# 16lemoing/waldo

Measured on AMD Instinct MI355X. Metric: warped+composited frames/sec at 256x512, 8 layers; fwd+bwd, higher is better.
Workload: dtype f32; 1 GPU; C3: 8 clips x 14 frames per GPU, 8 layers x 4x256x512, 16 TPS control points, fwd+bwd; frames_per_gpu=112, layers=8, height=256, width=512, parallelism=frames sharded x1, no data-path collective

## Files before the change

waldo_amd/csrc/waldo_common.hip.h:

```cpp
#pragma once
#include <hip/hip_runtime.h>
#include <stdint.h>
#include <type_traits>

#include "../../include/waldo_hip.h"
#include "warp_composite_layout.hip.h"

namespace waldo {

void set_error(const char* fmt, ...);
int launch_status(const char* what);
bool debug_option(int option);

void fill_words(void* dst, unsigned word, size_t bytes, hipStream_t st);
void copy_bytes(void* dst, const void* src, size_t bytes, hipStream_t st);

constexpr int kWave = 64;
constexpr int kBlock = 256;

constexpr int kStatusCtx = 0, kStatusPred = 2;

__device__ __forceinline__ int checked_frame(const int64_t* __restrict__ ts, int64_t i, int limit,
                                             int* __restrict__ status, int slot) {
  const int64_t raw = ts[i];
// ... 27 lines not shown
  return kXcds / g;
}
__device__ __forceinline__ bool xcd_decode_banded(unsigned bid, int nA, int nbands, int nT, int inner,
                                                  int& a, int& tile, int& rest) {
  const int tpb = (nT + nbands - 1) / nbands;
  int unit, j;
  if (!xcd_decode(bid, nA * nbands, tpb * inner, unit, j)) return false;
  a = unit / nbands;
  const int t = j / inner;
  rest = j - t * inner;
  tile = (unit - a * nbands) * tpb + t;
  return tile < nT;
}
__host__ inline int64_t xcd_grid_banded(int64_t nA, int nbands, int64_t nT, int64_t inner) {
  return xcd_grid(nA * nbands, ((nT + nbands - 1) / nbands) * inner);
}

struct Taps {
  float w00, w01, w10, w11;
  uint32_t o00, o01, o10, o11;
  float fx, fy;
  float vx0, vx1, vy0, vy1;
  int x0, y0;
};

__device__ __forceinline__ float unnormalize(float c, int size) {
  return ((c + 1.0f) * (float)size - 1.0f) * 0.5f;
}

struct TapCore {
// ... 330 lines not shown
```

waldo_amd/csrc/warp_composite_bwd_px16.hip.h:

```cpp
#pragma once

namespace waldo {

__device__ __forceinline__ int pk_max_u16(int a, int b) {
  typedef unsigned short u2 __attribute__((ext_vector_type(2)));
  u2 x, y;
  __builtin_memcpy(&x, &a, 4);
  __builtin_memcpy(&y, &b, 4);
  u2 r = __builtin_elementwise_max(x, y);
  int o;
  __builtin_memcpy(&o, &r, 4);
  return o;
}

__device__ __forceinline__ int exponent_of(float v) { return (int)(__float_as_uint(v) >> 23) & 0xff; }

#ifndef WALDO_K1_STAGE_AHEAD
#define WALDO_K1_STAGE_AHEAD 3
#endif

template <int LP>
struct Px16Cfg {
  static constexpr int K3 = kGmapK3, KS = (K3 + 3) / 4;
  static constexpr int NC = 2 * LP, NT = (NC + 15) / 16, GGC = NT * 16, TP = GGC + 1;
// ... 15 lines not shown
  static constexpr int kStage1 = kBtEnd > kStage0 ? kBtEnd : kStage0;
  static constexpr int kStage2 = (!kPark && kAccFloats > kStage1) ? kAccFloats : kStage1;
  static constexpr int kStageFloats = (kStage2 + 3) / 4 * 4;
  static constexpr int kLdsFloats = kParkFloats + kStageFloats + 4 * GGC * 2 + 4 * LP;
  static constexpr int kWavesPerSimd = LP <= 8 ? 3 : 2;
};

template <int LP, bool EXL, bool GOCC, typename TL = float, bool DET = false>
__global__ __launch_bounds__(kBlock, (GOCC ? 2 : Px16Cfg<LP>::kWavesPerSimd)) void warp_composite_bwd_px16_kernel(
    const TL* __restrict__ layers, const float* __restrict__ basis_t,
    const float* __restrict__ mapping, const float* __restrict__ occ,
    const float* __restrict__ grad_rgb, const float* __restrict__ grad_alpha,
    float4* __restrict__ rec, int* __restrict__ cellbox,
    unsigned* __restrict__ cellbound, float* __restrict__ gmap_partial, float* __restrict__ grad_occ,
    int F, int Lrt, int H, int W, int frames_per_block, int ntx, int ntiles, int nchunks, int nbands,
    int ncx, int ncells, float delta) {
  typedef float f32x4 __attribute__((ext_vector_type(4)));
  using C = Px16Cfg<LP>;
  constexpr int K3 = C::K3, KS = C::KS, NT = C::NT, GGC = C::GGC, TP = C::TP, OP = C::OP;
  constexpr bool kPark = C::kPark;
  const int L = EXL ? LP : Lrt;
  const int64_t HW = (int64_t)H * W;
  const int lane = threadIdx.x & (kWave - 1), wave = __builtin_amdgcn_readfirstlane(threadIdx.x >> 6);
  const int arow = lane & 15, kk = lane >> 4;
  int chunk, tile, rest_;
  if (!xcd_decode_banded(blockIdx.x, nchunks, nbands, ntiles, 1, chunk, tile, rest_)) return;

  __shared__ __attribute__((aligned(16))) float lds[C::kLdsFloats];
  float* park = lds;
  float* img = lds + C::kParkFloats;
  float* gg = kPark ? park : img;
  float* boxred = img + C::kStageFloats;
  int* wbound = reinterpret_cast<int*>(boxred + 4 * GGC * 2);
  const int pix = threadIdx.x;

  const int col0 = (tile % ntx) * kLdsTile, row0 = (tile / ntx) * kLdsTile + wave * 4;
  const bool live = col0 + arow < W && row0 + kk < H;
  const float livef = live ? 1.0f : 0.0f;
  const int64_t p = (int64_t)min(row0 + kk, H - 1) * W + min(col0 + arow, W - 1);
  for (int i = threadIdx.x; i < C::kStageFloats; i += kBlock) img[i] = 0.0f;

  float av[4][KS];
#pragma unroll
  for (int g = 0; g < 4; ++g) {
    const uint32_t pa = (uint32_t)(min(row0 + g, H - 1) * W + min(col0 + arow, W - 1));
#pragma unroll
    for (int ks = 0; ks < KS; ++ks) {
      const int k = 4 * ks + kk;
      const float bs = ldb(basis_t, ((uint32_t)min(k, K3 - 1) * (uint32_t)HW + pa) * 4u);
      av[g][ks] = (k < K3) ? bs : 0.0f;
    }
  }
  __syncthreads();

  const float half_size = 0.5f * (float)((arow & 1) ? H : W);
  const float half_size_m1 = 0.5f * (float)(((arow & 1) ? H : W) - 1);
  const int f0 = chunk * frames_per_block;
  const int f1 = min(F, f0 + frames_per_block);
  const int lane_k = lane, arow_k = arow, kk_k = kk, pix_k = pix;
  for (int f = f0; f < f1; ++f) {
    int lane = lane_k, arow = arow_k, kk = kk_k, pix = pix_k;
    asm volatile("" : "+v"(lane), "+v"(arow), "+v"(kk), "+v"(pix));
    const float* oc = occ + (int64_t)f * L * L;
    f32x4 acc[4][NT];
#pragma unroll
    for (int g = 0; g < 4; ++g)
#pragma unroll
      for (int nt = 0; nt < NT; ++nt) acc[g][nt] = (f32x4){0.0f, 0.0f, 0.0f, 0.0f};
    const float* mp = mapping + (int64_t)f * L * K3 * 2;
    {
      float mraw[KS][NT];
#pragma unroll
      for (int ks = 0; ks < KS; ++ks)
// ... 98 lines not shown
        bw[l] = ((xmax - bx0[l] + 1) + 3) & ~3;
        bh[l] = ymax - ymin + 1;
        fits[l] = bh[l] * bw[l] <= kStageCap;
      }
    }

    WALDO_PRIO_ON(WALDO_K1_PRIO_MASK, 2);
    const float g0 = grad_rgb[(int64_t)f * 3 * HW + p] * livef;
    const float g1 = grad_rgb[(int64_t)f * 3 * HW + HW + p] * livef;
    const float g2 = grad_rgb[(int64_t)f * 3 * HW + 2 * HW + p] * livef;
    const float gsum = fabsf(g0) + fabsf(g1) + fabsf(g2);
    float a[LP], G[LP];
    float dxr[kPark ? 1 : LP], dxa[kPark ? 1 : LP], dyr[kPark ? 1 : LP], dya[kPark ? 1 : LP];

    constexpr int kAhead = LP < WALDO_K1_STAGE_AHEAD ? LP : WALDO_K1_STAGE_AHEAD;
    int item_l = threadIdx.x;
    asm volatile("" : "+v"(item_l));
    typename StageOf<TL>::type stg[LP];
    auto issue = [&](int l) {
      const int lc = EXL ? l : min(l, L - 1);
      const TL* src = layers + ((int64_t)f * L + lc) * 4 * HW;
      const int bw2 = bw[l] >> 1, n = fits[l] ? bh[l] * bw2 : 1;
      const int ox = fits[l] ? __mul24(by0[l], W) + bx0[l] : 0;
      const float rcp = __builtin_amdgcn_rcpf((float)bw2);
      const int item = min(item_l, n - 1);
      const int r = (int)(((float)item + 0.5f) * rcp);
      const int xh = item - __mul24(r, bw2);
      stage_load(stg[l], src, HW, (unsigned)(ox + __mul24(r, W) + 2 * xh));
    };
#pragma unroll
    for (int l = 0; l < kAhead; ++l) issue(l);
    WALDO_PRIO_OFF(WALDO_K1_PRIO_MASK, 2);
    {
#pragma unroll
      for (int l = 0; l < LP; ++l) {
        if (!EXL && l >= L) {
          a[l] = 0.0f;
          G[l] = 0.0f;
          if constexpr (kPark) {
            reinterpret_cast<f32x4*>(park)[l * kBlock + pix] = (f32x4){0.0f, 0.0f, 0.0f, 0.0f};
          } else {
            dxr[l] = dxa[l] = dyr[l] = dya[l] = 0.0f;
          }
          continue;
        }
        WALDO_PRIO_ON(WALDO_K1_PRIO_MASK, 1);
        if (fits[l]) {
          const int n = bh[l] * (bw[l] >> 1);
          if (item_l < n)
            stage_put<TL>(img + (l & 1) * kImgBufFloats, item_l, stg[l]);
        }
        if (l + kAhead < LP) issue(l + kAhead);
        WALDO_PRIO_OFF(WALDO_K1_PRIO_MASK, 1);
        float gal = 0.0f;
        if (grad_alpha != nullptr) gal = grad_alpha[((int64_t)f * L + l) * HW + p];
        __syncthreads();
        const TapCore tc = tap_core_px(gxs[l], gys[l], H, W);
        const float* b0 = img + (l & 1) * kImgBufFloats;
        float sv[4], sx[4], sy[4];
        if (!fits[l]) {
          const Taps tg = finish_taps(tc, H, W);
          const TL* base = layers + ((int64_t)f * L + l) * 4 * HW;
#pragma unroll
          for (int c = 0; c < 4; ++c) sv[c] = tap_sample_d(base + c * HW, tg, sx[c], sy[c], delta);
        } else {
// ... 271 lines not shown
```

waldo_amd/csrc/warp_composite_fwd_lds.hip.h:

```cpp
#pragma once

namespace waldo {

#ifndef WALDO_FWD12_WAVES
#define WALDO_FWD12_WAVES 4
#endif
#ifndef WALDO_FWD8_WAVES
#define WALDO_FWD8_WAVES 3
#endif
#ifndef WALDO_FWD_PRIO_MASK
#define WALDO_FWD_PRIO_MASK 0
#endif
#ifndef WALDO_K1_PRIO_MASK
#define WALDO_K1_PRIO_MASK 3
#endif
#define WALDO_PRIO_ON(mask, bit) do { if ((mask) & (bit)) __builtin_amdgcn_s_setprio(1); } while (0)
#define WALDO_PRIO_OFF(mask, bit) do { if ((mask) & (bit)) __builtin_amdgcn_s_setprio(0); } while (0)
#ifndef WALDO_STAGE_AHEAD
#define WALDO_STAGE_AHEAD 2
#endif

struct BoxTaps {
  float fx, fy;
  float v00, v01, v10, v11;
// ... 15 lines not shown
  p.cs = t.x0 - p.xb;
  p.rs = t.y0 - p.yb;
  return p;
}

__device__ __forceinline__ int block_origin(float i, int size) {
  i = __builtin_amdgcn_fmed3f(i, -2.0f, (float)size + 1.0f);
  return min(max((int)floorf(i), 0), size - 2);
}

typedef float f32x2_t __attribute__((ext_vector_type(2)));
typedef float f32x4_t __attribute__((ext_vector_type(4)));

constexpr int kImgBufFloats = 4 * kStageCap;

struct StageRegs {
  f32x2_t c0, c1, c2, c3;
};

__device__ __forceinline__ f32x2_t pk_lo(f32x2_t a, f32x2_t b) {
  f32x2_t d;
  asm("v_pk_mov_b32 %0, %1, %2 op_sel:[0,0]" : "=v"(d) : "v"(a), "v"(b));
  return d;
}
__device__ __forceinline__ f32x2_t pk_hi(f32x2_t a, f32x2_t b) {
  f32x2_t d;
  asm("v_pk_mov_b32 %0, %1, %2 op_sel:[1,1]" : "=v"(d) : "v"(a), "v"(b));
  return d;
}

__device__ __forceinline__ void stage_store(float* imgbuf, int item, const StageRegs& r) {
  f32x4_t* dst = reinterpret_cast<f32x4_t*>(imgbuf + 8 * item);
  dst[0] = __builtin_shufflevector(pk_lo(r.c0, r.c1), pk_lo(r.c2, r.c3), 0, 1, 2, 3);
  dst[1] = __builtin_shufflevector(pk_hi(r.c0, r.c1), pk_hi(r.c2, r.c3), 0, 1, 2, 3);
}

__device__ __forceinline__ f32x2_t ld8(const float* __restrict__ base, uint32_t byte_off) {
  return *reinterpret_cast<const f32x2_t*>(reinterpret_cast<const char*>(base) + byte_off);
}

struct StageRegs16 {
  uint32_t c0, c1, c2, c3;
};
template <typename T>
struct StageOf {
  typedef StageRegs16 type;
};
template <>
struct StageOf<float> {
  typedef StageRegs type;
};

template <typename T>
__device__ __forceinline__ f32x2_t widen2(uint32_t w) {
  if constexpr (std::is_same_v<T, __bf16>) {
    return (f32x2_t){__uint_as_float(w << 16), __uint_as_float(w & 0xffff0000u)};
  } else {
    typename Half2<T>::type h;
    __builtin_memcpy(&h, &w, 4);
    return __builtin_convertvector(h, f32x2_t);
  }
}

template <typename T>
__device__ __forceinline__ void stage_load(typename StageOf<T>::type& r, const T* __restrict__ src, int64_t HW,
                                           unsigned tex) {
  if constexpr (std::is_same_v<T, float>) {
    const unsigned off = tex * 4u;
    r.c0 = ld8(src, off);
    r.c1 = ld8(src + HW, off);
    r.c2 = ld8(src + 2 * HW, off);
    r.c3 = ld8(src + 3 * HW, off);
  } else {
    auto ld4 = [](const T* base, unsigned byte_off) {
      return *reinterpret_cast<const uint32_t*>(reinterpret_cast<const char*>(base) + byte_off);
    };
    const unsigned off = tex * 2u;
    r.c0 = ld4(src, off);
    r.c1 = ld4(src + HW, off);
    r.c2 = ld4(src + 2 * HW, off);
    r.c3 = ld4(src + 3 * HW, off);
  }
}

template <typename T>
__device__ __forceinline__ void stage_put(float* imgbuf, int item, const typename StageOf<T>::type& r) {
  if constexpr (std::is_same_v<T, float>) {
    stage_store(imgbuf, item, r);
  } else {
    StageRegs w;
    w.c0 = widen2<T>(r.c0);
    w.c1 = widen2<T>(r.c1);
    w.c2 = widen2<T>(r.c2);
    w.c3 = widen2<T>(r.c3);
    stage_store(imgbuf, item, w);
  }
}

struct PairBlock {
  f32x2_t p00[2], p01[2], p10[2], p11[2];
};

__device__ __forceinline__ PairBlock read_block(const float* imgbuf, int idx, int bw) {
  const f32x4_t* r0 = reinterpret_cast<const f32x4_t*>(imgbuf + 4 * idx);
  const f32x4_t* r1 = r0 + bw;
  const f32x4_t t00 = r0[0], t01 = r0[1], t10 = r1[0], t11 = r1[1];
  PairBlock b;
  b.p00[0] = __builtin_shufflevector(t00, t00, 0, 1);
  b.p00[1] = __builtin_shufflevector(t00, t00, 2, 3);
  b.p01[0] = __builtin_shufflevector(t01, t01, 0, 1);
  b.p01[1] = __builtin_shufflevector(t01, t01, 2, 3);
// ... 21 lines not shown

__device__ __forceinline__ f32x2_t lerp2(const f32x2_t p00, const f32x2_t p01, const f32x2_t p10,
                                         const f32x2_t p11, float fx, float fy) {
  const f32x2_t fx2 = {fx, fx}, fy2 = {fy, fy};
  const f32x2_t top = __builtin_elementwise_fma(fx2, p01 - p00, p00);
  const f32x2_t bot = __builtin_elementwise_fma(fx2, p11 - p10, p10);
  return __builtin_elementwise_fma(fy2, bot - top, top);
}

template <int LP, bool EXL, bool FOLD, int NW = 4, typename TL = float>
__global__ __launch_bounds__(NW * kWave, (NW == 8 ? 1 : 1) * (LP <= 8 ? WALDO_FWD8_WAVES : (LP <= 12 ? (EXL ? WALDO_FWD12_WAVES : 3) : 2))) void warp_composite_fwd_lds_kernel(
    const TL* __restrict__ layers, const float* __restrict__ basis_t,
    const float* __restrict__ mapping, const float* __restrict__ inv_kernel,
    const float* __restrict__ src_pts, const float* __restrict__ occ, float* __restrict__ rgb,
    float* __restrict__ alpha_out, int F, int Lrt, int H, int W, int frames_per_block, int ntx,
    int ntiles, int nchunks, int nbands, float delta) {
  typedef float f32x4 __attribute__((ext_vector_type(4)));
  constexpr int K3 = 19, KS = (K3 + 3) / 4;
  constexpr int NC = 2 * LP, NT = (NC + 15) / 16, GGC = NT * 16, TP = GGC + 1;
  constexpr int kThreads = NW * kWave, kCap = kStageCap * NW / 4, kBuf = 4 * kCap;
  constexpr int kImgFloats = 2 * kBuf;
  constexpr int kTFloats = NW * kWave * TP;
  constexpr int kMain = kImgFloats > kTFloats ? kImgFloats : kTFloats;
  const int L = EXL ? LP : Lrt;
  const int64_t HW = (int64_t)H * W;
  const int lane = threadIdx.x & (kWave - 1), wave = __builtin_amdgcn_readfirstlane(threadIdx.x >> 6);
  const int arow = lane & 15, kk = lane >> 4;
  int chunk, tile, rest_;
  if (!xcd_decode_banded(blockIdx.x, nchunks, nbands, ntiles, 1, chunk, tile, rest_)) return;
  const int col0 = (tile % ntx) * (kLdsTile * NW / 4) + (wave >> 2) * kLdsTile;
  const int row0 = (tile / ntx) * kLdsTile + (wave & 3) * 4;
  PixelMap pm;
  pm.live = col0 + arow < W && row0 + kk < H;
  pm.p = (int64_t)min(row0 + kk, H - 1) * W + min(col0 + arow, W - 1);
  const int64_t p = pm.p;

  constexpr int kMapFloats = FOLD ? 2 * LP * K3 * 2 : 0;
  __shared__ __attribute__((aligned(16))) float lds[kMain + NW * GGC * 2 + kMapFloats];
  float* img = lds;
  float* boxred = lds + kMain;
  float* smap = boxred + NW * GGC * 2;
  auto fold_mapping = [&](int fm) {
    if constexpr (FOLD) {
      for (int e = threadIdx.x; e < L * K3 * 2; e += kThreads) {
// ... 38 lines not shown
  };
  static_assert(kMain % 4 == 0, "cleared sixteen bytes at a time");
  for (int i = threadIdx.x; i < kMain / 4; i += kThreads) reinterpret_cast<f32x4*>(lds)[i] = (f32x4){0.0f, 0.0f, 0.0f, 0.0f};

  float av[4][KS];
#pragma unroll
  for (int g = 0; g < 4; ++g) {
    const uint32_t pa = (uint32_t)(min(row0 + g, H - 1) * W + min(col0 + arow, W - 1));
#pragma unroll
    for (int ks = 0; ks < KS; ++ks) {
      const int k = 4 * ks + kk;
      const float bs = ldb(basis_t, ((uint32_t)min(k, K3 - 1) * (uint32_t)HW + pa) * 4u);
      av[g][ks] = (k < K3) ? bs : 0.0f;
    }
  }
  const int f0 = chunk * frames_per_block;
  const int f1 = min(F, f0 + frames_per_block);
  if (f0 < f1) fold_first(f0);
  __syncthreads();

  const float half_size = 0.5f * (float)((arow & 1) ? H : W);
  const float half_size_m1 = 0.5f * (float)(((arow & 1) ? H : W) - 1);
  const int lane_k = lane, arow_k = arow, kk_k = kk;
  for (int f = f0; f < f1; ++f) {
    int lane = lane_k, arow = arow_k, kk = kk_k;
    asm volatile("" : "+v"(lane), "+v"(arow), "+v"(kk));
    f32x4 acc[4][NT];
#pragma unroll
    for (int g = 0; g < 4; ++g)
#pragma unroll
      for (int nt = 0; nt < NT; ++nt) acc[g][nt] = (f32x4){0.0f, 0.0f, 0.0f, 0.0f};
    const float* mp = FOLD ? smap + (f & 1) * (LP * K3 * 2) : mapping + (int64_t)f * L * K3 * 2;
// ... 76 lines not shown
      hi_t[nt] = block_origin(mx, size) + 1;
    }
    int bx0[LP], by0[LP], bw[LP], bh[LP];
#pragma unroll
    for (int l = 0; l < LP; ++l) {
      const int nt = (2 * l) / 16, ln = (2 * l) % 16;
      const int xmin = __builtin_amdgcn_readlane(lo_t[nt], ln), xmax = __builtin_amdgcn_readlane(hi_t[nt], ln);
      const int ymin = __builtin_amdgcn_readlane(lo_t[nt], ln + 1), ymax = __builtin_amdgcn_readlane(hi_t[nt], ln + 1);
      bx0[l] = xmin & ~3;
      by0[l] = ymin;
      bw[l] = ((xmax - bx0[l] + 1) + 3) & ~3;
      bh[l] = ymax - ymin + 1;
    }

    constexpr int kAhead = LP < WALDO_STAGE_AHEAD ? LP : WALDO_STAGE_AHEAD;
    static_assert(kCap / 2 == kThreads, "one box item per lane");
    int item_l = threadIdx.x;
    asm volatile("" : "+v"(item_l));
    float s[LP][4];
    typename StageOf<TL>::type stg[LP];
    auto issue = [&](int l) {
      const int lc = EXL ? l : min(l, L - 1);
      const TL* src = layers + ((int64_t)f * L + lc) * 4 * HW;
      const bool fits = bh[l] * bw[l] <= kCap;
      const int bw2 = bw[l] >> 1, n = fits ? bh[l] * bw2 : 1;
      const int ox = fits ? __mul24(by0[l], W) + bx0[l] : 0;
      const float rcp = __builtin_amdgcn_rcpf((float)bw2);
      const int item = min(item_l, n - 1);
      const int r = (int)(((float)item + 0.5f) * rcp);
      const int xh = item - __mul24(r, bw2);
      stage_load(stg[l], src, HW, (unsigned)(ox + __mul24(r, W) + 2 * xh));
    };
    WALDO_PRIO_ON(WALDO_FWD_PRIO_MASK, 2);
#pragma unroll
    for (int l = 0; l < kAhead; ++l) issue(l);
    WALDO_PRIO_OFF(WALDO_FWD_PRIO_MASK, 2);
    {
#pragma unroll
      for (int l = 0; l < LP; ++l) {
        if (!EXL && l >= L) {
          s[l][0] = s[l][1] = s[l][2] = 0.0f;
          s[l][3] = -1.0f;
          continue;
        }
        const bool fits = bh[l] * bw[l] <= kCap;
        WALDO_PRIO_ON(WALDO_FWD_PRIO_MASK, 1);
        if (fits) {
          const int n = bh[l] * (bw[l] >> 1);
          if (item_l < n)
            stage_put<TL>(img + (l & 1) * kBuf, item_l, stg[l]);
        }
        if (l + kAhead < LP) issue(l + kAhead);
        WALDO_PRIO_OFF(WALDO_FWD_PRIO_MASK, 1);
        __syncthreads();
        if (fits) {
          const TapCore tc = tap_core_px(gx[l], gy[l], H, W);
          const float* b0 = img + (l & 1) * kBuf;
          f32x2_t sv[2];
          if (__ballot(!tap_interior(tc, H, W)) == 0ull) {
            const int idx = __mul24(tc.y0 - by0[l], bw[l]) + (tc.x0 - bx0[l]);
            const PairBlock pb = read_block(b0, idx, bw[l]);
#pragma unroll
            for (int q = 0; q < 2; ++q) sv[q] = lerp2(pb.p00[q], pb.p01[q], pb.p10[q], pb.p11[q], tc.fx, tc.fy);
          } else {
            const BoxTaps t = make_box_taps(tc, H, W);
// ... 67 lines not shown
```

waldo_amd/csrc/warp_composite_kernels.hip.h:

```cpp
#pragma once
#include <stdlib.h>

#include <type_traits>

#include "waldo_common.hip.h"

namespace waldo {

constexpr int kMaxLayers = 32;
constexpr int kMaxK3 = 32;
constexpr int kFwdGroup = 4;
constexpr int kBwdGroup = 2;

template <int K3P, bool EXK>
__device__ __forceinline__ void load_basis(float (&bas)[K3P], const float* __restrict__ basis_t,
                                           int64_t HW, int64_t p, int K3) {
#pragma unroll
  for (int k = 0; k < K3P; ++k) {
    if constexpr (EXK) {
      bas[k] = basis_t[(int64_t)k * HW + p];
    } else {
      const int kc = min(k, K3 - 1);
      const float v = basis_t[(int64_t)kc * HW + p];
      bas[k] = (k < K3) ? v : 0.0f;
// ... 221 lines not shown
        const float ggy = giy * (0.5f * (float)H);
        float part[2 * K3P];
#pragma unroll
        for (int k = 0; k < K3P; ++k) {
          part[2 * k] = bas[k] * ggx;
          part[2 * k + 1] = bas[k] * ggy;
        }
        float red = wave_transpose_reduce<2 * K3P>(part, lane);
        int idx = bitrev6(lane);
        if (idx < 2 * K3) atomicAdd(grad_mapping + ((int64_t)f * L + l) * K3 * 2 + idx, red);
      }
    }
  }
}

constexpr int kRedOut = 32, kRedSlices = kBlock / kRedOut;

static __global__ __launch_bounds__(kBlock) void warp_composite_gmap_reduce_kernel(
    const float* __restrict__ gmap_partial, float* __restrict__ grad_mapping, int F, int L,
    int ntiles, int groups) {
  const int per = L * kGmapK3 * 2;
  const int64_t f = blockIdx.x / groups;
  const int o = (blockIdx.x % groups) * kRedOut + (threadIdx.x % kRedOut);
  const int slice = threadIdx.x / kRedOut;
  __shared__ float red[kRedSlices][kRedOut];
  float s0 = 0.0f, s1 = 0.0f;
  if (o < per) {
    const int t0 = (int)((int64_t)ntiles * slice / kRedSlices), t1 = (int)((int64_t)ntiles * (slice + 1) / kRedSlices);
    const float* src = gmap_partial + f * ntiles * per + o;
    int t = t0;
    for (; t + 1 < t1; t += 2) {
      s0 += src[(int64_t)t * per];
      s1 += src[(int64_t)(t + 1) * per];
    }
    if (t < t1) s0 += src[(int64_t)t * per];
  }
  red[slice][threadIdx.x % kRedOut] = s0 + s1;
  __syncthreads();
  if (slice == 0 && o < per) {
    float sum = 0.0f;
#pragma unroll
    for (int k = 0; k < kRedSlices; ++k) sum += red[k][threadIdx.x];
    grad_mapping[f * per + o] += sum;
  }
}

template <typename T>
void launch_splat(const float* rec, const float* grad_rgb, const int* cellbox,
                  const unsigned* cellbound, T* grad_layers, int F, int L, int H, int W,
                  hipStream_t st);

}

#include "det_common.hip.h"
#include "warp_composite_fwd_lds.hip.h"
#include "warp_composite_bwd_px16.hip.h"

namespace waldo {

static inline int chunk_frames(int F, int64_t ntiles) {
  for (int c = 8; c >= 2; --c) {
    const int chunks = (F + c - 1) / c;
    if (chunks % kXcds == 0 && (int64_t)chunks * ntiles >= 2048) return c;
  }
  return 1;
}

struct TileGeom {
  int ntx, nty, ntiles;
};

static inline TileGeom tile_geom(int H, int W, int rows) {
  TileGeom g;
  g.ntx = (W + kTileW - 1) / kTileW;
  g.nty = (H + rows - 1) / rows;
  g.ntiles = g.ntx * g.nty;
  return g;
}

#ifndef WALDO_FWD_NW
// ... 3 lines not shown
static void launch_fwd(const T* layers, const float* basis_t, const float* mapping,
                       const float* inv_kernel, const float* src_pts,
                       const float* occ, float* rgb, float* alpha, int F, int L, int H, int W,
                       int K3, float delta, hipStream_t st) {
  constexpr bool kF32 = std::is_same_v<T, float>;
  const TileGeom g = tile_geom(H, W, 4);
  const int fpb = chunk_frames(F, g.ntiles);
  const int nchunks = (F + fpb - 1) / fpb;
  const int nbands = xcd_bands(nchunks);
  dim3 grid((unsigned)xcd_grid_banded(nchunks, nbands, g.ntiles, 1));
  if constexpr (EXK) {
    if (!kF32 || (!debug_option(WALDO_DEBUG_FWD_PLAIN) && staged_eligible(H, W))) {
      constexpr int NW = (WALDO_FWD_NW == 8 && LP <= 12) ? 8 : 4;
      constexpr int TW = kLdsTile * NW / 4;
      const int ntx16 = (W + TW - 1) / TW, nt16 = ntx16 * ((H + kLdsTile - 1) / kLdsTile);
      dim3 grid16((unsigned)xcd_grid_banded(nchunks, nbands, nt16, 1));
      auto go = [&](auto exl, auto fold) {
        constexpr bool EXL = decltype(exl)::value, FOLD = decltype(fold)::value;
        hipLaunchKernelGGL((warp_composite_fwd_lds_kernel<LP, EXL, FOLD, NW, T>), grid16, dim3(NW * kWave), 0, st, layers,
                           basis_t, mapping, inv_kernel, src_pts, occ, rgb, alpha, F, L, H, W, fpb, ntx16, nt16,
                           nchunks, nbands, delta);
      };
      using Y = std::true_type;
      using N = std::false_type;
      if (src_pts != nullptr) {
        if (L == LP) go(Y{}, Y{}); else go(N{}, Y{});
      } else {
        if (L == LP) go(Y{}, N{}); else go(N{}, N{});
      }
      return;
    }
  }
  if constexpr (kF32) {
    if (L == LP)
      hipLaunchKernelGGL((warp_composite_fwd_kernel<LP, K3P, true, EXK>), grid, dim3(kBlock), 0, st,
                         layers, basis_t, mapping, occ, rgb, alpha, F, L, H, W, K3, fpb, g.ntx, g.ntiles,
// ... 25 lines not shown
                        int F, int L, int H, int W, float delta, hipStream_t st, float* occ_slab = nullptr) {
  const Bwd2Layout lo = bwd2_layout(F, L, H, W);
  char* ws = reinterpret_cast<char*>(workspace);
  int* boxes = reinterpret_cast<int*>(ws);
  unsigned* bounds = reinterpret_cast<unsigned*>(ws + lo.box_bytes);
  float4* rec = reinterpret_cast<float4*>(ws + lo.box_bytes + lo.bound_bytes);
  float* part = grad_mapping == nullptr
                    ? nullptr
                    : reinterpret_cast<float*>(ws + lo.box_bytes + lo.bound_bytes + lo.rec_bytes);
  using Y = std::true_type;
  using N = std::false_type;
  const int ntiles = lo.ntiles16;
  const int fpb = chunk_frames(F, ntiles);
  const int nchunks = (F + fpb - 1) / fpb;
  const int nbands = xcd_bands(nchunks);
  dim3 grid((unsigned)xcd_grid_banded(nchunks, nbands, ntiles, 1));
  auto go = [&](auto exl, auto gocc) {
    constexpr bool EXL = decltype(exl)::value, GOCC = decltype(gocc)::value;
    hipLaunchKernelGGL((warp_composite_bwd_px16_kernel<LP, EXL, GOCC, T>), grid, dim3(kBlock), 0, st, layers,
                       basis_t, mapping, occ, grad_rgb, grad_alpha, rec, boxes, bounds, part,
                       grad_occ, F, L, H, W, fpb, lo.ntx16, ntiles, nchunks, nbands, lo.ncx, lo.ncells,
                       delta);
  };
  if (grad_occ != nullptr && occ_slab != nullptr) {
    auto go_det = [&](auto exl) {
      hipLaunchKernelGGL((warp_composite_bwd_px16_kernel<LP, decltype(exl)::value, true, T, true>), grid, dim3(kBlock), 0,
                         st, layers, basis_t, mapping, occ, grad_rgb, grad_alpha, rec, boxes, bounds, part, occ_slab, F,
                         L, H, W, fpb, lo.ntx16, ntiles, nchunks, nbands, lo.ncx, lo.ncells, delta);
    };
    if (L == LP) go_det(Y{}); else go_det(N{});
    slab_reduce(occ_slab, grad_occ, F, ntiles * 4, L * L, SlabPlain{(int64_t)F * ntiles * 4, F, F}, st);
  } else if (L == LP) {
    if (grad_occ != nullptr) go(Y{}, Y{}); else go(Y{}, N{});
  } else {
    if (grad_occ != nullptr) go(N{}, Y{}); else go(N{}, N{});
  }
  if (part != nullptr) {
    const int groups = (int)((gmap_partial_floats(L) + kRedOut - 1) / kRedOut);
    hipLaunchKernelGGL(warp_composite_gmap_reduce_kernel, dim3((unsigned)((int64_t)F * groups)), dim3(kBlock),
                       0, st, part, grad_mapping, F, L, ntiles, groups);
  }
  launch_splat<T>(reinterpret_cast<const float*>(rec), grad_rgb, boxes, bounds, grad_layers, F, L, H, W, st);
}

}
```

waldo_amd/csrc/warp_composite_splat.hip:

```cpp
#include <type_traits>

#include "waldo_common.hip.h"

namespace waldo {

#ifndef WALDO_K2_COLS
#define WALDO_K2_COLS 64
#endif
#ifndef WALDO_K2_WAVES
#define WALDO_K2_WAVES 8
#endif
#ifndef WALDO_K2_ROWS
#define WALDO_K2_ROWS 32
#endif
constexpr int kSrcRows = WALDO_K2_ROWS, kSrcCols = WALDO_K2_COLS;
constexpr int kColShift = kSrcCols == 64 ? 6 : 5;
static_assert((1 << kColShift) == kSrcCols, "S tile: 32 or 64 columns");
constexpr int kSrcTex = kSrcRows * kSrcCols;
constexpr int kCellPix = kCellRows * kCellCols;
constexpr int kCellShift = kCellPix == 64 ? 6 : (kCellPix == 128 ? 7 : 8);
static_assert((1 << kCellShift) == kCellPix, "cell rows: 4, 8 or 16");
constexpr int kG2Waves = WALDO_K2_WAVES;
constexpr int kG2Threads = kG2Waves * kWave;
constexpr int kMaxHit = 192 * 8 / kCellRows;
// ... 70 lines not shown
    const f32x2 g0s = {gv[2 * q], gv[2 * q]}, g1s = {gv[2 * q + 1], gv[2 * q + 1]};
    const f32x2 pt0 = g0s * wt_rgb, pb0 = g0s * wb_rgb;
    const f32x2 pt1 = g1s * (q == 0 ? wt_rgb : wt_a), pb1 = g1s * (q == 0 ? wb_rgb : wb_a);
    add2(a00, q, pt0[0], pt1[0]);
    add2(a01, q, pt0[1], pt1[1]);
    add2(a10, q, pb0[0], pb1[0]);
    add2(a11, q, pb0[1], pb1[1]);
  }
}

__device__ __forceinline__ bool touches(const TapCore& t, int sx0, int sy0) {
  const int lx0 = t.x0 - sx0, ly0 = t.y0 - sy0;
  return lx0 >= -1 && lx0 < kSrcCols && ly0 >= -1 && ly0 < kSrcRows;
}

template <typename T>
__global__ __launch_bounds__(kG2Threads, 2) void warp_composite_splat_kernel(
    const float4* __restrict__ rec, const float* __restrict__ grad_rgb,
    const int* __restrict__ cellbox, const unsigned* __restrict__ cellbound,
    T* __restrict__ grad_layers, int F, int L, int H, int W, int nsx, int nstiles, int nbands,
    int ncx, int ncells) {
  const int64_t HW = (int64_t)H * W;
  const int lane = threadIdx.x & (kWave - 1), wave = threadIdx.x >> 6;
  int fi, stile, layer;
  if (!xcd_decode_banded(blockIdx.x, F, nbands, nstiles, L, fi, stile, layer)) return;
  const int64_t f = fi;
  const int64_t fl = f * L + layer;
  const int sx0 = (stile % nsx) * kSrcCols, sy0 = (stile / nsx) * kSrcRows;
  const int sx1 = min(sx0 + kSrcCols, W) - 1, sy1 = min(sy0 + kSrcRows, H) - 1;

  __shared__ __attribute__((aligned(16))) int lds[4 * kPlane + kMaxHit + kScanPer * kG2Waves + 5 * kSubs];
  int* img = lds;
  int* hitlist = lds + 4 * kPlane;
  int* wcount = hitlist + kMaxHit;
  int* sbcnt = wcount + kScanPer * kG2Waves;
  unsigned* sbmax = reinterpret_cast<unsigned*>(sbcnt + kSubs);
  f32x2_k2* sbscale = reinterpret_cast<f32x2_k2*>(sbmax + 2 * kSubs);
  static_assert((4 * kPlane + kMaxHit + kScanPer * kG2Waves + 3 * kSubs) % 2 == 0, "8-byte aligned scale table");


  auto reaches = [&](const int4 ob) {
    return (bool)((ob.x <= ob.y) & (ob.x <= sx1) & (ob.y >= sx0) & (ob.z <= sy1) & (ob.w >= sy0));
  };
  int nhit = 0;
  const float cell_rows = (float)kCellRows;
  for (int c0 = 0; c0 < ncells; c0 += kScanPer * kG2Threads) {
// ... 257 lines not shown
      const int li = (e >> kColShift) * kPitch + (e & (kSrcCols - 1));
      const f32x2_k2 sc = sbscale[((y - sy0) >> 3) * kSubX + ((x - sx0) >> 4)];
#pragma unroll
      for (int c = 0; c < 4; ++c) {
        const int lo = img[2 * ((c >> 1) * kPlane + li)], hi = img[2 * ((c >> 1) * kPlane + li) + 1];
        const int v = (c & 1) ? hi - (lo >> 31) : lo;
        (gbase + c * HW)[doff] = (T)((float)v * __uint_as_float(0x7f000000u - __float_as_uint(sc[c < 3 ? 0 : 1])));
      }
    }
  }
}

template <typename T>
void launch_splat(const float* rec, const float* grad_rgb, const int* cellbox,
                  const unsigned* cellbound, T* grad_layers, int F, int L, int H, int W,
                  hipStream_t st) {
  const int nsx = (W + kSrcCols - 1) / kSrcCols, nsy = (H + kSrcRows - 1) / kSrcRows;
  const int ncx = (W + kCellCols - 1) / kCellCols, ncy = (H + kCellRows - 1) / kCellRows;
  const int nbands = xcd_bands(F);
  dim3 grid((unsigned)xcd_grid_banded(F, nbands, nsx * nsy, L));
  hipLaunchKernelGGL(warp_composite_splat_kernel<T>, grid, dim3(kG2Threads), 0, st,
                     reinterpret_cast<const float4*>(rec),
                     grad_rgb, cellbox, cellbound, grad_layers, F, L, H, W, nsx, nsx * nsy, nbands, ncx,
                     ncx * ncy);
}

template void launch_splat<float>(const float*, const float*, const int*, const unsigned*, float*, int, int, int, int,
                                  hipStream_t);
template void launch_splat<__bf16>(const float*, const float*, const int*, const unsigned*, __bf16*, int, int, int,
                                   int, hipStream_t);
template void launch_splat<_Float16>(const float*, const float*, const int*, const unsigned*, _Float16*, int, int, int,
                                     int, hipStream_t);

}
```

Before: 35630 frames/s.

## Split tail chunks into single-frame blocks, widen staging loads, fuse gmap reduce into splat

Adds a tailed grid decode so that, in the last chunk per XCD, some tiles run as one-frame work items. This is meant to even out the end-of-grid imbalance in the forward and backward kernels. Staging now uses half the workgroup per channel pair with 16-byte quad loads instead of 8-byte pair loads, which cuts load instruction count. The separate gmap reduction kernel is folded into extra blocks of the splat launch, removing one kernel launch. The risks are more blocks and a possible LDS pattern change in the stage stores.

```diff
diff --git a/waldo_amd/csrc/waldo_common.hip.h b/waldo_amd/csrc/waldo_common.hip.h
--- a/waldo_amd/csrc/waldo_common.hip.h
+++ b/waldo_amd/csrc/waldo_common.hip.h
@@ -65,6 +65,37 @@
 }
 __host__ inline int64_t xcd_grid_banded(int64_t nA, int nbands, int64_t nT, int64_t inner) {
   return xcd_grid(nA * nbands, ((nT + nbands - 1) / nbands) * inner);
+}
+
+__host__ inline int64_t xcd_grid_tailed(int nchunks, int nbands, int64_t ntiles, int fpb, int ntail, int tail_frames) {
+  if (ntail == 0) return xcd_grid_banded(nchunks, nbands, ntiles, 1);
+  const int nsub = (fpb + tail_frames - 1) / tail_frames;
+  return kXcds * ((int64_t)(nchunks / kXcds) * ntiles + (int64_t)ntail * (nsub - 1));
+}
+__device__ __forceinline__ bool xcd_decode_tailed(unsigned bid, int nchunks, int nbands, int ntiles, int fpb, int ntail,
+                                                  int tail_frames, int F, int& tile, int& f0, int& f1) {
+  if (ntail == 0) {
+    int chunk, rest;
+    if (!xcd_decode_banded(bid, nchunks, nbands, ntiles, 1, chunk, tile, rest)) return false;
+    f0 = chunk * fpb;
+    f1 = min(F, f0 + fpb);
+    return true;
+  }
+  const int xcd = (int)(bid & (kXcds - 1)), j = (int)(bid >> 3);
+  const int cpx = nchunks / kXcds, bulk = cpx * ntiles - ntail;
+  if (j < bulk) {
+    const int al = j / ntiles;
+    tile = j - al * ntiles;
+    f0 = (al * kXcds + xcd) * fpb;
+    f1 = min(F, f0 + fpb);
+  } else {
+    const int jj = j - bulk, sub = jj / ntail;
+    tile = ntiles - ntail + (jj - sub * ntail);
+    const int c0 = ((cpx - 1) * kXcds + xcd) * fpb;
+    f0 = c0 + sub * tail_frames;
+    f1 = min(F, min(f0 + tail_frames, c0 + fpb));
+  }
+  return f0 < f1;
 }
 
 struct Taps {
diff --git a/waldo_amd/csrc/warp_composite_bwd_px16.hip.h b/waldo_amd/csrc/warp_composite_bwd_px16.hip.h
--- a/waldo_amd/csrc/warp_composite_bwd_px16.hip.h
+++ b/waldo_amd/csrc/warp_composite_bwd_px16.hip.h
@@ -53,7 +53,7 @@
     float4* __restrict__ rec, int* __restrict__ cellbox,
     unsigned* __restrict__ cellbound, float* __restrict__ gmap_partial, float* __restrict__ grad_occ,
     int F, int Lrt, int H, int W, int frames_per_block, int ntx, int ntiles, int nchunks, int nbands,
-    int ncx, int ncells, float delta) {
+    int ncx, int ncells, int ntail, int tail_frames, float delta) {
   typedef float f32x4 __attribute__((ext_vector_type(4)));
   using C = Px16Cfg<LP>;
   constexpr int K3 = C::K3, KS = C::KS, NT = C::NT, GGC = C::GGC, TP = C::TP, OP = C::OP;
@@ -62,8 +62,8 @@
   const int64_t HW = (int64_t)H * W;
   const int lane = threadIdx.x & (kWave - 1), wave = __builtin_amdgcn_readfirstlane(threadIdx.x >> 6);
   const int arow = lane & 15, kk = lane >> 4;
-  int chunk, tile, rest_;
-  if (!xcd_decode_banded(blockIdx.x, nchunks, nbands, ntiles, 1, chunk, tile, rest_)) return;
+  int tile, f0, f1;
+  if (!xcd_decode_tailed(blockIdx.x, nchunks, nbands, ntiles, frames_per_block, ntail, tail_frames, F, tile, f0, f1)) return;
 
   __shared__ __attribute__((aligned(16))) float lds[C::kLdsFloats];
   float* park = lds;
@@ -94,8 +94,6 @@
 
   const float half_size = 0.5f * (float)((arow & 1) ? H : W);
   const float half_size_m1 = 0.5f * (float)(((arow & 1) ? H : W) - 1);
-  const int f0 = chunk * frames_per_block;
-  const int f1 = min(F, f0 + frames_per_block);
   const int lane_k = lane, arow_k = arow, kk_k = kk, pix_k = pix;
   for (int f = f0; f < f1; ++f) {
     int lane = lane_k, arow = arow_k, kk = kk_k, pix = pix_k;
@@ -224,19 +222,21 @@
     float dxr[kPark ? 1 : LP], dxa[kPark ? 1 : LP], dyr[kPark ? 1 : LP], dya[kPark ? 1 : LP];
 
     constexpr int kAhead = LP < WALDO_K1_STAGE_AHEAD ? LP : WALDO_K1_STAGE_AHEAD;
-    int item_l = threadIdx.x;
+    static_assert(kStageCap / 4 == kBlock / 2, "one box item per lane of half the workgroup");
+    const int pair = wave >> 1;
+    int item_l = threadIdx.x & (kBlock / 2 - 1);
     asm volatile("" : "+v"(item_l));
-    typename StageOf<TL>::type stg[LP];
+    StageRegs<TL> stg[LP];
     auto issue = [&](int l) {
       const int lc = EXL ? l : min(l, L - 1);
-      const TL* src = layers + ((int64_t)f * L + lc) * 4 * HW;
-      const int bw2 = bw[l] >> 1, n = fits[l] ? bh[l] * bw2 : 1;
+      const TL* src = layers + (((int64_t)f * L + lc) * 4 + 2 * pair) * HW;
+      const int bw4 = bw[l] >> 2, n = fits[l] ? bh[l] * bw4 : 1;
       const int ox = fits[l] ? __mul24(by0[l], W) + bx0[l] : 0;
-      const float rcp = __builtin_amdgcn_rcpf((float)bw2);
+      const float rcp = __builtin_amdgcn_rcpf((float)bw4);
       const int item = min(item_l, n - 1);
       const int r = (int)(((float)item + 0.5f) * rcp);
-      const int xh = item - __mul24(r, bw2);
-      stage_load(stg[l], src, HW, (unsigned)(ox + __mul24(r, W) + 2 * xh));
+      const int xq = item - __mul24(r, bw4);
+      stage_load(stg[l], src, HW, (unsigned)(ox + __mul24(r, W) + 4 * xq));
     };
 #pragma unroll
     for (int l = 0; l < kAhead; ++l) issue(l);
@@ -256,9 +256,9 @@
         }
         WALDO_PRIO_ON(WALDO_K1_PRIO_MASK, 1);
         if (fits[l]) {
-          const int n = bh[l] * (bw[l] >> 1);
+          const int n = bh[l] * (bw[l] >> 2);
           if (item_l < n)
-            stage_put<TL>(img + (l & 1) * kImgBufFloats, item_l, stg[l]);
+            stage_put<TL>(img + (l & 1) * kImgBufFloats, item_l, pair, stg[l]);
         }
         if (l + kAhead < LP) issue(l + kAhead);
         WALDO_PRIO_OFF(WALDO_K1_PRIO_MASK, 1);
diff --git a/waldo_amd/csrc/warp_composite_fwd_lds.hip.h b/waldo_amd/csrc/warp_composite_fwd_lds.hip.h
--- a/waldo_amd/csrc/warp_composite_fwd_lds.hip.h
+++ b/waldo_amd/csrc/warp_composite_fwd_lds.hip.h
@@ -53,10 +53,6 @@
 
 constexpr int kImgBufFloats = 4 * kStageCap;
 
-struct StageRegs {
-  f32x2_t c0, c1, c2, c3;
-};
-
 __device__ __forceinline__ f32x2_t pk_lo(f32x2_t a, f32x2_t b) {
   f32x2_t d;
   asm("v_pk_mov_b32 %0, %1, %2 op_sel:[0,0]" : "=v"(d) : "v"(a), "v"(b));
@@ -67,28 +63,6 @@
   asm("v_pk_mov_b32 %0, %1, %2 op_sel:[1,1]" : "=v"(d) : "v"(a), "v"(b));
   return d;
 }
-
-__device__ __forceinline__ void stage_store(float* imgbuf, int item, const StageRegs& r) {
-  f32x4_t* dst = reinterpret_cast<f32x4_t*>(imgbuf + 8 * item);
-  dst[0] = __builtin_shufflevector(pk_lo(r.c0, r.c1), pk_lo(r.c2, r.c3), 0, 1, 2, 3);
-  dst[1] = __builtin_shufflevector(pk_hi(r.c0, r.c1), pk_hi(r.c2, r.c3), 0, 1, 2, 3);
-}
-
-__device__ __forceinline__ f32x2_t ld8(const float* __restrict__ base, uint32_t byte_off) {
-  return *reinterpret_cast<const f32x2_t*>(reinterpret_cast<const char*>(base) + byte_off);
-}
-
-struct StageRegs16 {
-  uint32_t c0, c1, c2, c3;
-};
-template <typename T>
-struct StageOf {
-  typedef StageRegs16 type;
-};
-template <>
-struct StageOf<float> {
-  typedef StageRegs type;
-};
 
 template <typename T>
 __device__ __forceinline__ f32x2_t widen2(uint32_t w) {
@@ -101,39 +75,48 @@
   }
 }
 
-template <typename T>
-__device__ __forceinline__ void stage_load(typename StageOf<T>::type& r, const T* __restrict__ src, int64_t HW,
-                                           unsigned tex) {
+typedef uint32_t u32x2_t __attribute__((ext_vector_type(2)));
+template <typename T>
+struct QuadOf {
+  typedef u32x2_t type;
+};
+template <>
+struct QuadOf<float> {
+  typedef f32x4_t type;
+};
+template <typename T>
+struct StageRegs {
+  typename QuadOf<T>::type c[2];
+};
+
+template <typename T>
+__device__ __forceinline__ void stage_load(StageRegs<T>& r, const T* __restrict__ src, int64_t HW, unsigned tex) {
+  const unsigned off = tex * (unsigned)sizeof(T);
+#pragma unroll
+  for (int i = 0; i < 2; ++i)
+    r.c[i] = *reinterpret_cast<const typename QuadOf<T>::type*>(reinterpret_cast<const char*>(src + i * HW) + off);
+}
+
+template <typename T>
+__device__ __forceinline__ f32x4_t widen4(const typename QuadOf<T>::type& q) {
   if constexpr (std::is_same_v<T, float>) {
-    const unsigned off = tex * 4u;
-    r.c0 = ld8(src, off);
-    r.c1 = ld8(src + HW, off);
-    r.c2 = ld8(src + 2 * HW, off);
-    r.c3 = ld8(src + 3 * HW, off);
+    return q;
   } else {
-    auto ld4 = [](const T* base, unsigned byte_off) {
-      return *reinterpret_cast<const uint32_t*>(reinterpret_cast<const char*>(base) + byte_off);
-    };
-    const unsigned off = tex * 2u;
-    r.c0 = ld4(src, off);
-    r.c1 = ld4(src + HW, off);
-    r.c2 = ld4(src + 2 * HW, off);
-    r.c3 = ld4(src + 3 * HW, off);
+    return __builtin_shufflevector(widen2<T>(q[0]), widen2<T>(q[1]), 0, 1, 2, 3);
   }
 }
 
-template <typename T>
-__device__ __forceinline__ void stage_put(float* imgbuf, int item, const typename StageOf<T>::type& r) {
-  if constexpr (std::is_same_v<T, float>) {
-    stage_store(imgbuf, item, r);
-  } else {
-    StageRegs w;
-    w.c0 = widen2<T>(r.c0);
-    w.c1 = widen2<T>(r.c1);
-    w.c2 = widen2<T>(r.c2);
-    w.c3 = widen2<T>(r.c3);
-    stage_store(imgbuf, item, w);
-  }
+__device__ __forceinline__ f32x2_t lo2(f32x4_t v) { return __builtin_shufflevector(v, v, 0, 1); }
+__device__ __forceinline__ f32x2_t hi2(f32x4_t v) { return __builtin_shufflevector(v, v, 2, 3); }
+
+template <typename T>
+__device__ __forceinline__ void stage_put(float* imgbuf, int item, int pair, const StageRegs<T>& r) {
+  const f32x4_t wa = widen4<T>(r.c[0]), wb = widen4<T>(r.c[1]);
+  f32x2_t* dst = reinterpret_cast<f32x2_t*>(imgbuf + 16 * item + 2 * pair);
+  dst[0] = pk_lo(lo2(wa), lo2(wb));
+  dst[2] = pk_hi(lo2(wa), lo2(wb));
+  dst[4] = pk_lo(hi2(wa), hi2(wb));
+  dst[6] = pk_hi(hi2(wa), hi2(wb));
 }
 
 struct PairBlock {
@@ -185,7 +168,7 @@
     const float* __restrict__ mapping, const float* __restrict__ inv_kernel,
     const float* __restrict__ src_pts, const float* __restrict__ occ, float* __restrict__ rgb,
     float* __restrict__ alpha_out, int F, int Lrt, int H, int W, int frames_per_block, int ntx,
-    int ntiles, int nchunks, int nbands, float delta) {
+    int ntiles, int nchunks, int nbands, int ntail, int tail_frames, float delta) {
   typedef float f32x4 __attribute__((ext_vector_type(4)));
   constexpr int K3 = 19, KS = (K3 + 3) / 4;
   constexpr int NC = 2 * LP, NT = (NC + 15) / 16, GGC = NT * 16, TP = GGC + 1;
@@ -197,8 +180,8 @@
   const int64_t HW = (int64_t)H * W;
   const int lane = threadIdx.x & (kWave - 1), wave = __builtin_amdgcn_readfirstlane(threadIdx.x >> 6);
   const int arow = lane & 15, kk = lane >> 4;
-  int chunk, tile, rest_;
-  if (!xcd_decode_banded(blockIdx.x, nchunks, nbands, ntiles, 1, chunk, tile, rest_)) return;
+  int tile, f0, f1;
+  if (!xcd_decode_tailed(blockIdx.x, nchunks, nbands, ntiles, frames_per_block, ntail, tail_frames, F, tile, f0, f1)) return;
   const int col0 = (tile % ntx) * (kLdsTile * NW / 4) + (wave >> 2) * kLdsTile;
   const int row0 = (tile / ntx) * kLdsTile + (wave & 3) * 4;
   PixelMap pm;
@@ -267,8 +250,6 @@
       av[g][ks] = (k < K3) ? bs : 0.0f;
     }
   }
-  const int f0 = chunk * frames_per_block;
-  const int f1 = min(F, f0 + frames_per_block);
   if (f0 < f1) fold_first(f0);
   __syncthreads();
 
@@ -375,22 +356,24 @@
     }
 
     constexpr int kAhead = LP < WALDO_STAGE_AHEAD ? LP : WALDO_STAGE_AHEAD;
-    static_assert(kCap / 2 == kThreads, "one box item per lane");
-    int item_l = threadIdx.x;
+    constexpr int kStagers = kThreads / 2;
+    static_assert(kCap / 4 == kStagers, "one box item per lane of half the workgroup");
+    const int pair = wave >= NW / 2 ? 1 : 0;
+    int item_l = threadIdx.x & (kStagers - 1);
     asm volatile("" : "+v"(item_l));
     float s[LP][4];
-    typename StageOf<TL>::type stg[LP];
+    StageRegs<TL> stg[LP];
     auto issue = [&](int l) {
       const int lc = EXL ? l : min(l, L - 1);
-      const TL* src = layers + ((int64_t)f * L + lc) * 4 * HW;
+      const TL* src = layers + (((int64_t)f * L + lc) * 4 + 2 * pair) * HW;
       const bool fits = bh[l] * bw[l] <= kCap;
-      const int bw2 = bw[l] >> 1, n = fits ? bh[l] * bw2 : 1;
+      const int bw4 = bw[l] >> 2, n = fits ? bh[l] * bw4 : 1;
       const int ox = fits ? __mul24(by0[l], W) + bx0[l] : 0;
-      const float rcp = __builtin_amdgcn_rcpf((float)bw2);
+      const float rcp = __builtin_amdgcn_rcpf((float)bw4);
       const int item = min(item_l, n - 1);
       const int r = (int)(((float)item + 0.5f) * rcp);
-      const int xh = item - __mul24(r, bw2);
-      stage_load(stg[l], src, HW, (unsigned)(ox + __mul24(r, W) + 2 * xh));
+      const int xq = item - __mul24(r, bw4);
+      stage_load(stg[l], src, HW, (unsigned)(ox + __mul24(r, W) + 4 * xq));
     };
     WALDO_PRIO_ON(WALDO_FWD_PRIO_MASK, 2);
 #pragma unroll
@@ -407,9 +390,9 @@
         const bool fits = bh[l] * bw[l] <= kCap;
         WALDO_PRIO_ON(WALDO_FWD_PRIO_MASK, 1);
         if (fits) {
-          const int n = bh[l] * (bw[l] >> 1);
+          const int n = bh[l] * (bw[l] >> 2);
           if (item_l < n)
-            stage_put<TL>(img + (l & 1) * kBuf, item_l, stg[l]);
+            stage_put<TL>(img + (l & 1) * kBuf, item_l, pair, stg[l]);
         }
         if (l + kAhead < LP) issue(l + kAhead);
         WALDO_PRIO_OFF(WALDO_FWD_PRIO_MASK, 1);
diff --git a/waldo_amd/csrc/warp_composite_kernels.hip.h b/waldo_amd/csrc/warp_composite_kernels.hip.h
--- a/waldo_amd/csrc/warp_composite_kernels.hip.h
+++ b/waldo_amd/csrc/warp_composite_kernels.hip.h
@@ -259,41 +259,10 @@
   }
 }
 
-constexpr int kRedOut = 32, kRedSlices = kBlock / kRedOut;
-
-static __global__ __launch_bounds__(kBlock) void warp_composite_gmap_reduce_kernel(
-    const float* __restrict__ gmap_partial, float* __restrict__ grad_mapping, int F, int L,
-    int ntiles, int groups) {
-  const int per = L * kGmapK3 * 2;
-  const int64_t f = blockIdx.x / groups;
-  const int o = (blockIdx.x % groups) * kRedOut + (threadIdx.x % kRedOut);
-  const int slice = threadIdx.x / kRedOut;
-  __shared__ float red[kRedSlices][kRedOut];
-  float s0 = 0.0f, s1 = 0.0f;
-  if (o < per) {
-    const int t0 = (int)((int64_t)ntiles * slice / kRedSlices), t1 = (int)((int64_t)ntiles * (slice + 1) / kRedSlices);
-    const float* src = gmap_partial + f * ntiles * per + o;
-    int t = t0;
-    for (; t + 1 < t1; t += 2) {
-      s0 += src[(int64_t)t * per];
-      s1 += src[(int64_t)(t + 1) * per];
-    }
-    if (t < t1) s0 += src[(int64_t)t * per];
-  }
-  red[slice][threadIdx.x % kRedOut] = s0 + s1;
-  __syncthreads();
-  if (slice == 0 && o < per) {
-    float sum = 0.0f;
-#pragma unroll
-    for (int k = 0; k < kRedSlices; ++k) sum += red[k][threadIdx.x];
-    grad_mapping[f * per + o] += sum;
-  }
-}
-
 template <typename T>
 void launch_splat(const float* rec, const float* grad_rgb, const int* cellbox,
                   const unsigned* cellbound, T* grad_layers, int F, int L, int H, int W,
-                  hipStream_t st);
+                  const float* gmap_partial, float* grad_mapping, int ntiles16, hipStream_t st);
 
 }
 
@@ -309,6 +278,27 @@
     if (chunks % kXcds == 0 && (int64_t)chunks * ntiles >= 2048) return c;
   }
   return 1;
+}
+
+#ifndef WALDO_TAIL_DIV
+#define WALDO_TAIL_DIV 8
+#endif
+#ifndef WALDO_TAIL_FRAMES
+#define WALDO_TAIL_FRAMES 1
+#endif
+struct ChunkTail {
+  int ntail, frames;
+  int64_t grid;
+};
+static inline ChunkTail chunk_tail(int nchunks, int nbands, int fpb, int64_t ntiles) {
+  ChunkTail t = {0, fpb, 0};
+  if (WALDO_TAIL_DIV > 0 && nbands == 1 && nchunks % kXcds == 0 && fpb > WALDO_TAIL_FRAMES) {
+    const int64_t want = (int64_t)(nchunks / kXcds) * ntiles / WALDO_TAIL_DIV;
+    t.ntail = (int)(want < ntiles ? want : ntiles);
+    t.frames = WALDO_TAIL_FRAMES;
+  }
+  t.grid = xcd_grid_tailed(nchunks, nbands, ntiles, fpb, t.ntail, t.frames);
+  return t;
 }
 
 struct TileGeom {
@@ -342,12 +332,13 @@
       constexpr int NW = (WALDO_FWD_NW == 8 && LP <= 12) ? 8 : 4;
       constexpr int TW = kLdsTile * NW / 4;
       const int ntx16 = (W + TW - 1) / TW, nt16 = ntx16 * ((H + kLdsTile - 1) / kLdsTile);
-      dim3 grid16((unsigned)xcd_grid_banded(nchunks, nbands, nt16, 1));
+      const ChunkTail ct = chunk_tail(nchunks, nbands, fpb, nt16);
+      dim3 grid16((unsigned)ct.grid);
       auto go = [&](auto exl, auto fold) {
         constexpr bool EXL = decltype(exl)::value, FOLD = decltype(fold)::value;
         hipLaunchKernelGGL((warp_composite_fwd_lds_kernel<LP, EXL, FOLD, NW, T>), grid16, dim3(NW * kWave), 0, st, layers,
                            basis_t, mapping, inv_kernel, src_pts, occ, rgb, alpha, F, L, H, W, fpb, ntx16, nt16,
-                           nchunks, nbands, delta);
+                           nchunks, nbands, ct.ntail, ct.frames, delta);
       };
       using Y = std::true_type;
       using N = std::false_type;
@@ -403,19 +394,20 @@
   const int fpb = chunk_frames(F, ntiles);
   const int nchunks = (F + fpb - 1) / fpb;
   const int nbands = xcd_bands(nchunks);
-  dim3 grid((unsigned)xcd_grid_banded(nchunks, nbands, ntiles, 1));
+  const ChunkTail ct = chunk_tail(nchunks, nbands, fpb, ntiles);
+  dim3 grid((unsigned)ct.grid);
   auto go = [&](auto exl, auto gocc) {
     constexpr bool EXL = decltype(exl)::value, GOCC = decltype(gocc)::value;
     hipLaunchKernelGGL((warp_composite_bwd_px16_kernel<LP, EXL, GOCC, T>), grid, dim3(kBlock), 0, st, layers,
                        basis_t, mapping, occ, grad_rgb, grad_alpha, rec, boxes, bounds, part,
                        grad_occ, F, L, H, W, fpb, lo.ntx16, ntiles, nchunks, nbands, lo.ncx, lo.ncells,
-                       delta);
+                       ct.ntail, ct.frames, delta);
   };
   if (grad_occ != nullptr && occ_slab != nullptr) {
     auto go_det = [&](auto exl) {
       hipLaunchKernelGGL((warp_composite_bwd_px16_kernel<LP, decltype(exl)::value, true, T, true>), grid, dim3(kBlock), 0,
                          st, layers, basis_t, mapping, occ, grad_rgb, grad_alpha, rec, boxes, bounds, part, occ_slab, F,
-                         L, H, W, fpb, lo.ntx16, ntiles, nchunks, nbands, lo.ncx, lo.ncells, delta);
+                         L, H, W, fpb, lo.ntx16, ntiles, nchunks, nbands, lo.ncx, lo.ncells, ct.ntail, ct.frames, delta);
     };
     if (L == LP) go_det(Y{}); else go_det(N{});
     slab_reduce(occ_slab, grad_occ, F, ntiles * 4, L * L, SlabPlain{(int64_t)F * ntiles * 4, F, F}, st);
@@ -424,12 +416,8 @@
   } else {
     if (grad_occ != nullptr) go(N{}, Y{}); else go(N{}, N{});
   }
-  if (part != nullptr) {
-    const int groups = (int)((gmap_partial_floats(L) + kRedOut - 1) / kRedOut);
-    hipLaunchKernelGGL(warp_composite_gmap_reduce_kernel, dim3((unsigned)((int64_t)F * groups)), dim3(kBlock),
-                       0, st, part, grad_mapping, F, L, ntiles, groups);
-  }
-  launch_splat<T>(reinterpret_cast<const float*>(rec), grad_rgb, boxes, bounds, grad_layers, F, L, H, W, st);
-}
-
-}
+  launch_splat<T>(reinterpret_cast<const float*>(rec), grad_rgb, boxes, bounds, grad_layers, F, L, H, W, part,
+                  grad_mapping, ntiles, st);
+}
+
+}
diff --git a/waldo_amd/csrc/warp_composite_splat.hip b/waldo_amd/csrc/warp_composite_splat.hip
--- a/waldo_amd/csrc/warp_composite_splat.hip
+++ b/waldo_amd/csrc/warp_composite_splat.hip
@@ -108,12 +108,57 @@
   return lx0 >= -1 && lx0 < kSrcCols && ly0 >= -1 && ly0 < kSrcRows;
 }
 
+constexpr int kRedThreads = 256, kRedOut = 32, kRedSlices = kRedThreads / kRedOut;
+constexpr int kRedPerBlock = kG2Threads / kRedThreads;
+static_assert(kG2Threads % kRedThreads == 0, "whole reduction groups per workgroup");
+
+__host__ __device__ inline int gmap_reduce_groups(int L) { return (int)((gmap_partial_floats(L) + kRedOut - 1) / kRedOut); }
+
+__device__ __forceinline__ void gmap_reduce_block(const float* __restrict__ gmap_partial,
+                                                  float* __restrict__ grad_mapping, float* red, unsigned unit, int F,
+                                                  int L, int ntiles) {
+  const int per = L * kGmapK3 * 2, groups = gmap_reduce_groups(L);
+  const int sub = threadIdx.x / kRedThreads, tid = threadIdx.x % kRedThreads;
+  const int64_t grp = (int64_t)unit * kRedPerBlock + sub;
+  const bool on = grp < (int64_t)F * groups;
+  const int64_t f = grp / groups;
+  const int o = (int)(grp % groups) * kRedOut + (tid % kRedOut);
+  const int slice = tid / kRedOut;
+  float* myred = red + sub * (kRedSlices * kRedOut);
+  float s0 = 0.0f, s1 = 0.0f;
+  if (on && o < per) {
+    const int t0 = (int)((int64_t)ntiles * slice / kRedSlices), t1 = (int)((int64_t)ntiles * (slice + 1) / kRedSlices);
+    const float* src = gmap_partial + f * ntiles * per + o;
+    int t = t0;
+    for (; t + 1 < t1; t += 2) {
+      s0 += src[(int64_t)t * per];
+      s1 += src[(int64_t)(t + 1) * per];
+    }
+    if (t < t1) s0 += src[(int64_t)t * per];
+  }
+  myred[slice * kRedOut + tid % kRedOut] = s0 + s1;
+  __syncthreads();
+  if (on && slice == 0 && o < per) {
+    float sum = 0.0f;
+#pragma unroll
+    for (int k = 0; k < kRedSlices; ++k) sum += myred[k * kRedOut + tid];
+    grad_mapping[f * per + o] += sum;
+  }
+}
+
 template <typename T>
 __global__ __launch_bounds__(kG2Threads, 2) void warp_composite_splat_kernel(
     const float4* __restrict__ rec, const float* __restrict__ grad_rgb,
     const int* __restrict__ cellbox, const unsigned* __restrict__ cellbound,
     T* __restrict__ grad_layers, int F, int L, int H, int W, int nsx, int nstiles, int nbands,
-    int ncx, int ncells) {
+    int ncx, int ncells, const float* __restrict__ gmap_partial, float* __restrict__ grad_mapping, int ntiles16,
+    unsigned nsplat) {
+  __shared__ __attribute__((aligned(16))) int lds[4 * kPlane + kMaxHit + kScanPer * kG2Waves + 5 * kSubs];
+  static_assert(4 * kPlane >= kRedPerBlock * kRedSlices * kRedOut, "the reduction's slice sums fit the image");
+  if (blockIdx.x >= nsplat) {
+    gmap_reduce_block(gmap_partial, grad_mapping, reinterpret_cast<float*>(lds), blockIdx.x - nsplat, F, L, ntiles16);
+    return;
+  }
   const int64_t HW = (int64_t)H * W;
   const int lane = threadIdx.x & (kWave - 1), wave = threadIdx.x >> 6;
   int fi, stile, layer;
@@ -123,7 +168,6 @@
   const int sx0 = (stile % nsx) * kSrcCols, sy0 = (stile / nsx) * kSrcRows;
   const int sx1 = min(sx0 + kSrcCols, W) - 1, sy1 = min(sy0 + kSrcRows, H) - 1;
 
-  __shared__ __attribute__((aligned(16))) int lds[4 * kPlane + kMaxHit + kScanPer * kG2Waves + 5 * kSubs];
   int* img = lds;
   int* hitlist = lds + 4 * kPlane;
   int* wcount = hitlist + kMaxHit;
@@ -411,22 +455,24 @@
 template <typename T>
 void launch_splat(const float* rec, const float* grad_rgb, const int* cellbox,
                   const unsigned* cellbound, T* grad_layers, int F, int L, int H, int W,
-                  hipStream_t st) {
+                  const float* gmap_partial, float* grad_mapping, int ntiles16, hipStream_t st) {
   const int nsx = (W + kSrcCols - 1) / kSrcCols, nsy = (H + kSrcRows - 1) / kSrcRows;
   const int ncx = (W + kCellCols - 1) / kCellCols, ncy = (H + kCellRows - 1) / kCellRows;
   const int nbands = xcd_bands(F);
-  dim3 grid((unsigned)xcd_grid_banded(F, nbands, nsx * nsy, L));
+  const int64_t nsplat = xcd_grid_banded(F, nbands, nsx * nsy, L);
+  const int64_t nred = gmap_partial == nullptr ? 0 : ((int64_t)F * gmap_reduce_groups(L) + kRedPerBlock - 1) / kRedPerBlock;
+  dim3 grid((unsigned)(nsplat + nred));
   hipLaunchKernelGGL(warp_composite_splat_kernel<T>, grid, dim3(kG2Threads), 0, st,
                      reinterpret_cast<const float4*>(rec),
                      grad_rgb, cellbox, cellbound, grad_layers, F, L, H, W, nsx, nsx * nsy, nbands, ncx,
-                     ncx * ncy);
+                     ncx * ncy, gmap_partial, grad_mapping, ntiles16, (unsigned)nsplat);
 }
 
 template void launch_splat<float>(const float*, const float*, const int*, const unsigned*, float*, int, int, int, int,
-                                  hipStream_t);
+                                  const float*, float*, int, hipStream_t);
 template void launch_splat<__bf16>(const float*, const float*, const int*, const unsigned*, __bf16*, int, int, int,
-                                   int, hipStream_t);
+                                   int, const float*, float*, int, hipStream_t);
 template void launch_splat<_Float16>(const float*, const float*, const int*, const unsigned*, _Float16*, int, int, int,
-                                     int, hipStream_t);
-
-}
+                                     int, const float*, float*, int, hipStream_t);
+
+}
```

Result: slower. 35260 frames/s (-1.0%).
